# TheoBald200814/RGB-D-Instance-Segmentation

Hardware: AMD Instinct MI355X
Metric: NYUv2 640x480 RGB-D img/s (fwd+bwd) of the DGGM+E-DSAM hot path (higher is better)
Workload: dtype bf16

## Files before the change

rgb-d-instance-segmentation_amd/csrc/ratio_chain.hip:

```cpp
#include "ratio_common.hpp"

using namespace rgbd;
using namespace rgbd::rp;

namespace {

__global__ __launch_bounds__(256) void k_rp_fold(const char* __restrict__ blob, Layout L,
                                                 const float2* __restrict__ aff, int which, char* __restrict__ fold) {
  const int c = blockIdx.x;
  const int K = which == 1 ? STEM_K2 : STEM_C;
  const float* w = (const float*)(blob + (which == 1 ? L.w1f : L.w2f)) + (size_t)c * K;
  bf16_t* wo = (bf16_t*)(fold + (which == 1 ? FOLD_W1 : FOLD_W2)) + (size_t)c * K;
  const float2 a = aff[c];
  for (int k = threadIdx.x; k < K; k += 256) wo[k] = f32_to_bf16(w[k] * a.x);
  if (threadIdx.x == 0) {
    const float b = ((const float*)(blob + (which == 1 ? L.b1 : L.b2)))[c];
    ((float*)(fold + (which == 1 ? FOLD_B1 : FOLD_B2)))[c] = __builtin_fmaf(b, a.x, a.y);
  }
}

constexpr int C2W_PWP = 40;
constexpr size_t C2W_OFF_W1 = 0;
constexpr size_t C2W_OFF_W2 = C2W_OFF_W1 + (size_t)STEM_C * C2W_S1 * 2;
constexpr size_t C2W_OFF_W3 = C2W_OFF_W2 + (size_t)FUS_C * C2W_S2 * 2;
constexpr size_t C2W_OFF_W4 = C2W_OFF_W3 + (size_t)ATT_C * C2W_S3 * 2;
template <int PH> constexpr size_t c2w_off_b() {
  return PH == 0 ? C2W_OFF_W2 : C2W_OFF_W4 + (size_t)FUS_C * C2W_S4 * 2;
}
template <int PH> constexpr size_t c2w_off_aff() {
  return c2w_off_b<PH>() + (size_t)(STEM_C + FUS_C + ATT_C + FUS_C) * 4;
}
template <int PH> constexpr size_t c2w_off_patch() {
  return c2w_off_aff<PH>() + (size_t)(STEM_C + FUS_C) * 8;
}
template <int PH> constexpr size_t c2w_smem() { return c2w_off_patch<PH>() + (size_t)3 * C2W_PH * C2W_PWP * 2 + 16; }
static_assert(c2w_smem<1>() <= 163840, "chain v2 LDS budget");
constexpr size_t C2W_OFF_P8 = C2W_OFF_W3;
constexpr int C2W_P8 = 8 * 3 * C2W_PH * C2W_PWP;
static_assert(C2W_OFF_P8 + (size_t)C2W_P8 * 2 <= c2w_off_b<1>(), "phase-1 shifted patches fit W3 + W4");
static_assert(2 * c2w_smem<0>() <= 163840, "chain v2 phase 0: two workgroups per CU");

__device__ unsigned long long* g_c2_stamps = nullptr;
[[maybe_unused]] static bool c2_stamps_on = false;
__device__ __forceinline__ void c2_stamp(unsigned long long* st, long long idx) {
  __builtin_amdgcn_sched_barrier(0);
  const unsigned long long t = __builtin_amdgcn_s_memtime();
  if ((threadIdx.x & 63) == 0) st[idx] = t;
  __builtin_amdgcn_sched_barrier(0);
}

template <int PHASE, bool STAMPS = false>
__global__ __launch_bounds__(512, PHASE == 0 ? 4 : 2) void k_rp_chain_v2(const float* __restrict__ depth3, long long bstride, int B,
                                                     int H, int W, const char* __restrict__ blob, Layout L,
                                                     const float2* __restrict__ aff1, const float2* __restrict__ aff2,
                                                     const char* __restrict__ fold, float* __restrict__ slab,
                                                     bf16_t* __restrict__ att) {
  extern __shared__ __attribute__((aligned(16))) char smem[];
  const bf16_t* sW1 = (const bf16_t*)(smem + C2W_OFF_W1);
  const bf16_t* sW2 = (const bf16_t*)(smem + C2W_OFF_W2);
  const bf16_t* sW3 = (const bf16_t*)(smem + C2W_OFF_W3);
  const bf16_t* sW4 = (const bf16_t*)(smem + C2W_OFF_W4);
  float* sb = (float*)(smem + c2w_off_b<PHASE>());
  float* sb1 = sb;
  float* sb2 = sb1 + STEM_C;
  float* sb3 = sb2 + FUS_C;
  float* sb4 = sb3 + ATT_C;
  bf16_t* patch = (bf16_t*)(smem + c2w_off_patch<PHASE>());
  const int tid = threadIdx.x, lane = tid & 63, wave = tid >> 6;
  const int r = lane & 15, g = lane >> 4;
  {
    auto copy_rows = [&](size_t dst, size_t src, int rows, int k, int stride) {
      const int per = k / 8;
      for (int i = tid; i < rows * per; i += 512) {
        const int rr = i / per, q = i % per;
        *reinterpret_cast<uint4*>(smem + dst + ((size_t)rr * stride + 8 * q) * 2) =
            *reinterpret_cast<const uint4*>(blob + src + ((size_t)rr * k + 8 * q) * 2);
      }
    };
    auto copy_rows_p = [&](size_t dst, const char* base, int rows, int k, int stride) {
      const int per = k / 8;
      for (int i = tid; i < rows * per; i += 512) {
        const int rr = i / per, q = i % per;
        *reinterpret_cast<uint4*>(smem + dst + ((size_t)rr * stride + 8 * q) * 2) =
            *reinterpret_cast<const uint4*>(base + ((size_t)rr * k + 8 * q) * 2);
      }
    };
    if (PHASE == 0)
      copy_rows(C2W_OFF_W1, L.w1s, STEM_C, STEM_K2, C2W_S1);
    else
      copy_rows_p(C2W_OFF_W1, fold + FOLD_W1, STEM_C, STEM_K2, C2W_S1);
    if (PHASE >= 1) {
      if (PHASE == 2)
        copy_rows_p(C2W_OFF_W2, fold + FOLD_W2, FUS_C, STEM_C, C2W_S2);
      else
        copy_rows(C2W_OFF_W2, L.w2, FUS_C, STEM_C, C2W_S2);
    }
    if (PHASE == 2) {
      copy_rows(C2W_OFF_W3, L.w3, ATT_C, FUS_C, C2W_S3);
      copy_rows(C2W_OFF_W4, L.w4, FUS_C, ATT_C, C2W_S4);
    }
    for (int i = tid; i < STEM_C; i += 512)
      sb1[i] = PHASE == 0 ? ((const float*)(blob + L.b1))[i] : ((const float*)(fold + FOLD_B1))[i];
    for (int i = tid; i < FUS_C; i += 512)
      sb2[i] = PHASE == 2 ? ((const float*)(fold + FOLD_B2))[i] : ((const float*)(blob + L.b2))[i];
    for (int i = tid; i < ATT_C; i += 512) sb3[i] = ((const float*)(blob + L.b3))[i];
    for (int i = tid; i < FUS_C; i += 512) sb4[i] = ((const float*)(blob + L.b4))[i];
    for (int i = tid; i < 3 * C2W_PH * C2W_PWP; i += 512) patch[i] = 0;
    for (int i = tid; i < STEM_C * (C2W_S1 - STEM_K2); i += 512)
      ((bf16_t*)(smem + C2W_OFF_W1))[(i / (C2W_S1 - STEM_K2)) * C2W_S1 + STEM_K2 + i % (C2W_S1 - STEM_K2)] = 0;
  }
  constexpr int NST = PHASE == 0 ? 12 : 8;
  float ssum[NST], ssq[NST];
#pragma unroll
  for (int i = 0; i < NST; ++i) ssum[i] = ssq[i] = 0.f;
  const int tiles_x = (W + C2W_TW - 1) / C2W_TW, tiles_y = (H + C2W_TH - 1) / C2W_TH;
  const unsigned per = (unsigned)(tiles_x * tiles_y);
  const int ntiles = B * tiles_x * tiles_y;
  const long long HW = (long long)H * W;
  constexpr int PATCH_N = 3 * C2W_PH * C2W_PW, PATCH_PER = (PATCH_N + 511) / 512;
  float pre[PATCH_PER];
  const long long dbytes = ((long long)(B - 1) * bstride + 3 * HW) * 4;
  const bool dbuf = PHASE >= 1 && dbytes < (1ll << 31);
  const __amdgpu_buffer_rsrc_t drs = wt_rsrc(depth3, dbuf ? (int)dbytes : 0);
  auto fetch_patch = [&](int t) {
    const TileDec td = tile_dec((unsigned)t, per, (unsigned)tiles_x, C2W_TH, C2W_TW);
#pragma unroll
    for (int k = 0; k < PATCH_PER; ++k) {
      const int i = tid + 512 * k;
      const int c = i / (C2W_PH * C2W_PW), yy = (i / C2W_PW) % C2W_PH, xx = i % C2W_PW;
      const int yv = td.y0 + yy - 3, xv = td.x0 + xx - 3;
      const bool ok = i < PATCH_N && t < ntiles && yv >= 0 && yv < H && xv >= 0 && xv < W;
      if (dbuf) {
        const uint32_t off = ok ? (uint32_t)((td.b * bstride + c * HW + (long long)yv * W + xv) * 4) : 0x80000000u;
        pre[k] = __uint_as_float(__builtin_amdgcn_raw_buffer_load_b32(drs, off, 0, 0));
      } else {
        float v = 0.f;
        if (ok) v = depth3[td.b * bstride + c * HW + (long long)yv * W + xv];
        pre[k] = v;
      }
    }
  };
  auto add_stats = [&](float& sm, float& sq, const f32x4 (&a)[2], bool full, int x0, bool row_ok) {
#pragma unroll
    for (int u = 0; u < 2; ++u)
#pragma unroll
      for (int j = 0; j < 4; ++j) {
        float v = a[u][j];
        if (!full) v = (row_ok && x0 + 16 * u + 4 * g + j < W) ? v : 0.f;
        sm += v;
        sq = __builtin_fmaf(v, v, sq);
      }
  };
  fetch_patch(blockIdx.x);
  int tcount = 0;
  for (int tile = blockIdx.x; tile < ntiles; tile += gridDim.x, ++tcount) {
    unsigned long long* const sts = (STAMPS && blockIdx.x == 0 && tcount >= 8 && tcount < 12) ? g_c2_stamps : nullptr;
    const long long sidx = ((long long)PHASE * 32 + (long long)(tcount - 8) * 8 + wave) * 7;
    if (STAMPS && sts) c2_stamp(sts, sidx + 0);
    const TileDec td = tile_dec((unsigned)tile, per, (unsigned)tiles_x, C2W_TH, C2W_TW);
    const int b = td.b, y0 = td.y0, x0 = td.x0;
    lds_barrier();
#pragma unroll
    for (int k = 0; k < PATCH_PER; ++k) {
      const int i = tid + 512 * k;
      if (i < PATCH_N) patch[(i / C2W_PW) * C2W_PWP + i % C2W_PW] = f32_to_bf16(pre[k]);
    }
    lds_barrier();
    if constexpr (PHASE == 1) {
      bf16_t* p8 = (bf16_t*)(smem + C2W_OFF_P8);
      for (int i = tid; i < 8 * 3 * C2W_PH * 4; i += 512) {
        const int j8 = i & 3, row = (i >> 2) % (3 * C2W_PH), k = i / (3 * C2W_PH * 4);
        const int e = 8 * j8 + k;
        const uint32_t* wp = reinterpret_cast<const uint32_t*>(patch + row * C2W_PWP + (e & ~1));
        const uint32_t w0 = wp[0], w1 = wp[1], w2 = wp[2], w3 = wp[3], w4 = wp[4];
        const uint32_t sh = (e & 1) * 2;
        *reinterpret_cast<uint4*>(p8 + (k * 3 * C2W_PH + row) * C2W_PWP + 8 * j8) =
            make_uint4(__builtin_amdgcn_alignbyte(w1, w0, sh), __builtin_amdgcn_alignbyte(w2, w1, sh),
                       __builtin_amdgcn_alignbyte(w3, w2, sh), __builtin_amdgcn_alignbyte(w4, w3, sh));
      }
      lds_barrier();
    }
    if (STAMPS && sts) c2_stamp(sts, sidx + 1);
    fetch_patch(tile + gridDim.x);
    if (STAMPS && sts) c2_stamp(sts, sidx + 2);
    const int py = y0 + wave;
    const bool row_ok = py < H;
    const bool full = row_ok && x0 + C2W_TW <= W;
    bool pv[2];
#pragma unroll
    for (int u = 0; u < 2; ++u) pv[u] = row_ok && x0 + 16 * u + r < W;
    auto stem_b = [&](int s, Frag<bf16_t> (&bf)[2]) {
      const int q = 4 * s + g;
      if constexpr (PHASE == 1) {
        const int qc = q < 21 ? q : 20;
        const int cq = qc / 7, dy = qc - 7 * cq;
        const bf16_t* p8 = (const bf16_t*)(smem + C2W_OFF_P8) + (((r & 7) * 3 + cq) * C2W_PH + wave + dy) * C2W_PWP +
                           (r & 8);
        bf[0].v = *reinterpret_cast<const uint4*>(p8);
        bf[1].v = *reinterpret_cast<const uint4*>(p8 + 16);
        if (q >= 21) {
          bf[0].zero();
          bf[1].zero();
        }
        return;
      }
      const int cq = q / 7, dy = q - 7 * cq;
#pragma unroll
      for (int u = 0; u < 2; ++u) {
        if (q < 21) {
          const int col = 16 * u + r;
          const uint32_t* wp = reinterpret_cast<const uint32_t*>(patch + (cq * C2W_PH + wave + dy) * C2W_PWP + (col & ~1));
          const uint32_t w0 = wp[0], w1 = wp[1], w2 = wp[2], w3 = wp[3], w4 = wp[4];
          const uint32_t sh = (col & 1) * 2;
          bf[u].v = make_uint4(__builtin_amdgcn_alignbyte(w1, w0, sh), __builtin_amdgcn_alignbyte(w2, w1, sh),
                               __builtin_amdgcn_alignbyte(w3, w2, sh), __builtin_amdgcn_alignbyte(w4, w3, sh));
        } else {
          bf[u].zero();
        }
      }
    };
    auto stem_w = [&](int t, int s) {
      Frag<bf16_t> af;
      af.v = *reinterpret_cast<const uint4*>(sW1 + (16 * t + r) * C2W_S1 + 32 * s + 8 * g);
      if (s == 5) af.select(g == 0);
      return af;
    };
    auto stem_live = [](int t, int s) { return !((t < 4 && (s == 3 || s == 5)) || (t >= 4 && t < 8 && s == 5)); };
    if constexpr (PHASE == 0) {
      Frag<bf16_t> bfr[6][2];
#pragma unroll
      for (int s = 0; s < 6; ++s) stem_b(s, bfr[s]);
#pragma unroll
      for (int t = 0; t < 12; ++t) {
        const float bb = sb1[16 * t + r];
        f32x4 a1[2] = {f32x4{bb, bb, bb, bb}, f32x4{bb, bb, bb, bb}};
#pragma unroll
        for (int s = 0; s < 6; ++s) {
          if (!stem_live(t, s)) continue;
          const Frag<bf16_t> af = stem_w(t, s);
          mma(a1[0], bfr[s][0], af);
          mma(a1[1], bfr[s][1], af);
        }
        add_stats(ssum[t], ssq[t], a1, full, x0, row_ok);
      }
      if (STAMPS && sts) c2_stamp(sts, sidx + 3);
      continue;
    }
    f32x4 a1[12][2];
#pragma unroll
    for (int t = 0; t < 12; ++t) {
      const float4 bb = *reinterpret_cast<const float4*>(sb1 + 16 * t + 4 * g);
      a1[t][0] = a1[t][1] = f32x4{bb.x, bb.y, bb.z, bb.w};
    }
    if constexpr (PHASE == 1) {
      Frag<bf16_t> bcur[2], bnxt[2];
      stem_b(0, bcur);
#pragma unroll
      for (int s = 0; s < 6; ++s) {
        if (s < 5) stem_b(s + 1, bnxt);
#pragma unroll
        for (int t = 0; t < 12; ++t) {
          if (!stem_live(t, s)) continue;
          const Frag<bf16_t> af = stem_w(t, s);
          mma(a1[t][0], af, bcur[0]);
          mma(a1[t][1], af, bcur[1]);
        }
        __builtin_amdgcn_sched_barrier(0);
        bcur[0] = bnxt[0];
        bcur[1] = bnxt[1];
      }
    } else {
#pragma unroll
      for (int s = 0; s < 6; ++s) {
        Frag<bf16_t> bfr[2];
        stem_b(s, bfr);
#pragma unroll
        for (int t = 0; t < 12; ++t) {
          if (!stem_live(t, s)) continue;
          const Frag<bf16_t> af = stem_w(t, s);
          mma(a1[t][0], af, bfr[0]);
          mma(a1[t][1], af, bfr[1]);
        }
      }
    }
    if (STAMPS && sts) c2_stamp(sts, sidx + 3);
    Frag<bf16_t> f1[6][2];
#pragma unroll
    for (int s = 0; s < 6; ++s)
#pragma unroll
      for (int u = 0; u < 2; ++u) {
        float vv[8];
#pragma unroll
        for (int e = 0; e < 8; ++e) vv[e] = fmaxf(a1[2 * s + (e >> 2)][u][e & 3], 0.f);
        f1[s][u].from8(vv);
      }
    if (STAMPS && sts) c2_stamp(sts, sidx + 4);
    f32x4 a2[8][2];
#pragma unroll
    for (int t = 0; t < 8; ++t) {
      if constexpr (PHASE == 1) {
        const float bb = sb2[16 * t + r];
        a2[t][0] = a2[t][1] = f32x4{bb, bb, bb, bb};
      } else {
        const float4 bb = *reinterpret_cast<const float4*>(sb2 + 16 * t + 4 * g);
        a2[t][0] = a2[t][1] = f32x4{bb.x, bb.y, bb.z, bb.w};
      }
#pragma unroll
      for (int s = 0; s < 6; ++s) {
        Frag<bf16_t> af;
        af.v = *reinterpret_cast<const uint4*>(sW2 + (16 * t + r) * C2W_S2 + 32 * s + 8 * g);
        if constexpr (PHASE == 1) {
          mma(a2[t][0], f1[s][0], af);
          mma(a2[t][1], f1[s][1], af);
        } else {
          mma(a2[t][0], af, f1[s][0]);
          mma(a2[t][1], af, f1[s][1]);
        }
      }
    }
    if (STAMPS && sts) c2_stamp(sts, sidx + 5);
    if constexpr (PHASE == 1) {
#pragma unroll
      for (int t = 0; t < 8; ++t) add_stats(ssum[t], ssq[t], a2[t], full, x0, row_ok);
      if (att) {
        bf16_t* ft = att + (((long long)tile * 8 + wave) * 16) * 256;
#pragma unroll
        for (int t = 0; t < 8; ++t)
          *reinterpret_cast<uint4*>(ft + (t * 64 + lane) * 8) =
              make_uint4(pack_bf16x2(a2[t][0][0], a2[t][0][1]), pack_bf16x2(a2[t][0][2], a2[t][0][3]),
                         pack_bf16x2(a2[t][1][0], a2[t][1][1]), pack_bf16x2(a2[t][1][2], a2[t][1][3]));
      }
      if (STAMPS && sts) c2_stamp(sts, sidx + 6);
      continue;
    }
    if constexpr (PHASE == 2) {
#pragma unroll
      for (int t = 0; t < 8; ++t)
#pragma unroll
        for (int j = 0; j < 4; ++j) {
          a2[t][0][j] = fmaxf(a2[t][0][j], 0.f);
          a2[t][1][j] = fmaxf(a2[t][1][j], 0.f);
        }
      Frag<bf16_t> f2[4][2];
#pragma unroll
      for (int s = 0; s < 4; ++s)
#pragma unroll
        for (int u = 0; u < 2; ++u) {
          float vv[8];
#pragma unroll
          for (int e = 0; e < 8; ++e) vv[e] = a2[2 * s + (e >> 2)][u][e & 3];
          f2[s][u].from8(vv);
        }
      f32x4 a3[4][2];
#pragma unroll
      for (int t = 0; t < 4; ++t) {
        const float4 bb = *reinterpret_cast<const float4*>(sb3 + 16 * t + 4 * g);
        a3[t][0] = a3[t][1] = f32x4{bb.x, bb.y, bb.z, bb.w};
#pragma unroll
        for (int s = 0; s < 4; ++s) {
          Frag<bf16_t> af;
          af.v = *reinterpret_cast<const uint4*>(sW3 + (16 * t + r) * C2W_S3 + 32 * s + 8 * g);
          mma(a3[t][0], af, f2[s][0]);
          mma(a3[t][1], af, f2[s][1]);
        }
      }
      Frag<bf16_t> f3[2][2];
#pragma unroll
      for (int s = 0; s < 2; ++s)
#pragma unroll
        for (int u = 0; u < 2; ++u) {
          float vv[8];
#pragma unroll
          for (int e = 0; e < 8; ++e) vv[e] = fmaxf(a3[2 * s + (e >> 2)][u][e & 3], 0.f);
          f3[s][u].from8(vv);
        }
#pragma unroll
      for (int t = 0; t < 8; ++t) {
        const float4 bb = *reinterpret_cast<const float4*>(sb4 + 16 * t + 4 * g);
        f32x4 a4[2] = {f32x4{bb.x, bb.y, bb.z, bb.w}, f32x4{bb.x, bb.y, bb.z, bb.w}};
#pragma unroll
        for (int s = 0; s < 2; ++s) {
          Frag<bf16_t> af;
          af.v = *reinterpret_cast<const uint4*>(sW4 + (16 * t + r) * C2W_S4 + 32 * s + 8 * g);
          mma(a4[0], af, f3[s][0]);
          mma(a4[1], af, f3[s][1]);
        }
#pragma unroll
        for (int u = 0; u < 2; ++u) {
          if (!pv[u]) continue;
          float o[4];
#pragma unroll
          for (int j = 0; j < 4; ++j) o[j] = a2[t][u][j] * sigmoid_fast(a4[u][j]);
          *reinterpret_cast<uint2*>(att + c4_att_idx(b, t >> 1, py, x0 + 16 * u + r, H, W) + 16 * (t & 1) + 4 * g) =
              make_uint2(pack_bf16x2(o[0], o[1]), pack_bf16x2(o[2], o[3]));
        }
      }
    }
  }
  if constexpr (PHASE < 2) {
    const long long row = (long long)blockIdx.x * 8 + wave;
    constexpr int NC = PHASE == 0 ? STEM_C : FUS_C;
#pragma unroll
    for (int t = 0; t < NST; ++t) {
      float a = ssum[t], q = ssq[t];
      a += __shfl_xor(a, 16);
      q += __shfl_xor(q, 16);
      a += __shfl_xor(a, 32);
      q += __shfl_xor(q, 32);
      if (g == 0) {
        const long long e = PHASE == 1 ? (long long)(16 * t + r) * (gridDim.x * 8) + row : row * NC + 16 * t + r;
        slab[e * 2 + 0] = a;
        slab[e * 2 + 1] = q;
      }
    }
  }
}

template <int PH>
int chain_launch(const float* depth3, long long bstride, int B, int H, int W, const char* blob, const Layout& L,
                 const float2* aff1, const float2* aff2, const char* fold, float* slab, bf16_t* att, hipStream_t s) {
  static const hipError_t attr = hipFuncSetAttribute((const void*)k_rp_chain_v2<PH>,
                                                     hipFuncAttributeMaxDynamicSharedMemorySize, (int)c2w_smem<PH>());
  if (attr != hipSuccess) return (int)attr;
  const int grid = chain_grid_v2(B, H, W, PH);
#ifdef RGBD_DIAG
  if constexpr (PH < 2) {
    if (c2_stamps_on) {
      static const hipError_t sattr = hipFuncSetAttribute(
          (const void*)k_rp_chain_v2<PH, true>, hipFuncAttributeMaxDynamicSharedMemorySize, (int)c2w_smem<PH>());
      (void)sattr;
      k_rp_chain_v2<PH, true><<<grid, 512, c2w_smem<PH>(), s>>>(depth3, bstride, B, H, W, blob, L, aff1, aff2, fold,
                                                               slab, att);
      return RGBD_OK;
    }
  }
#endif
  k_rp_chain_v2<PH><<<grid, 512, c2w_smem<PH>(), s>>>(depth3, bstride, B, H, W, blob, L, aff1, aff2, fold, slab, att);
  return RGBD_OK;
}

}

namespace rgbd::rp {

int chain_grid_v2(int B, int H, int W, int phase) {
  const long long nt = (long long)B * ((W + C2W_TW - 1) / C2W_TW) * ((H + C2W_TH - 1) / C2W_TH);
  return (int)std::min<long long>(nt, phase == 0 ? 512 : 256);
}

int fold_bn(const char* blob, const Layout& L, const float2* aff, int which, char* fold, hipStream_t s) {
  k_rp_fold<<<which == 1 ? STEM_C : FUS_C, 256, 0, s>>>(blob, L, aff, which, fold);
  return RGBD_OK;
}

int chain_v2(int phase, const float* depth3, long long bstride, int B, int H, int W, const char* blob, const Layout& L,
             const float2* aff1, const float2* aff2, const char* fold, float* slab, bf16_t* att, hipStream_t s) {
  if (phase == 0) return chain_launch<0>(depth3, bstride, B, H, W, blob, L, aff1, aff2, fold, slab, att, s);
  if (phase == 1) return chain_launch<1>(depth3, bstride, B, H, W, blob, L, aff1, aff2, fold, slab, att, s);
  TimerScope ts("rp_chain", s);
  return chain_launch<2>(depth3, bstride, B, H, W, blob, L, aff1, aff2, fold, slab, att, s);
}

}

#ifdef RGBD_DIAG
extern "C" int rgbd_debug_chain_stamps(void* buf) {
  unsigned long long* p = (unsigned long long*)buf;
  const hipError_t e = hipMemcpyToSymbol(HIP_SYMBOL(g_c2_stamps), &p, sizeof(p));
  if (e != hipSuccess) return (int)e;
  c2_stamps_on = p != nullptr;
  return RGBD_OK;
}
#endif
```

rgb-d-instance-segmentation_amd/csrc/ratio_conv5.hip:

```cpp
#include "ratio_common.hpp"

using namespace rgbd;
using namespace rgbd::rp;

namespace {

constexpr int GT_S = FUS_C + 8;
constexpr size_t GT_OFF_W3 = 0;
constexpr size_t GT_OFF_W4 = GT_OFF_W3 + (size_t)ATT_C * C2W_S3 * 2;
constexpr size_t GT_OFF_B = GT_OFF_W4 + (size_t)FUS_C * C2W_S4 * 2;
constexpr size_t GT_OFF_IMG = GT_OFF_B + (size_t)(ATT_C + FUS_C + 2 * FUS_C) * 4;
constexpr size_t GT_SMEM = GT_OFF_IMG + (size_t)8 * C2W_TW * GT_S * 2;
static_assert(GT_SMEM <= 163840, "gate LDS budget");

__global__ __launch_bounds__(512) void k_rp_gate(const bf16_t* __restrict__ fus, int B, int H, int W,
                                                 const char* __restrict__ blob, Layout L,
                                                 const float2* __restrict__ aff2, bf16_t* __restrict__ att) {
  extern __shared__ __attribute__((aligned(16))) char smem[];
  const bf16_t* sW3 = (const bf16_t*)(smem + GT_OFF_W3);
  const bf16_t* sW4 = (const bf16_t*)(smem + GT_OFF_W4);
  float* sb3 = (float*)(smem + GT_OFF_B);
  float* sb4 = sb3 + ATT_C;
  float2* saff = (float2*)(sb4 + FUS_C);
  const int tid = threadIdx.x, lane = tid & 63, wave = tid >> 6;
// ... 480 lines not shown
            const float lo = __uint_as_float(w[2 * h + e] << 16), hi = __uint_as_float(w[2 * h + e] & 0xffff0000u);
            acc[nh][h] += fmaxf(lo * af[nh][h].x + af[nh][h].y, 0.f);
            acc[nh][h] += fmaxf(hi * af[nh][h].x + af[nh][h].y, 0.f);
          }
      }
    }
  }
#pragma unroll
  for (int nh = 0; nh < 2; ++nh)
#pragma unroll
    for (int h = 0; h < 2; ++h) {
      float v = acc[nh][h];
      v += __shfl_xor(v, 16);
      v += __shfl_xor(v, 32);
      if (lane < 16) red[nh * 128 + 32 * np + 16 * h + r] = v;
    }
  __syncthreads();
  part[(((long long)b * 16 + reg) * POOL_SPLIT + sp) * C5 + t] = red[t];
}

__global__ __launch_bounds__(256) void k_rp_bn_relu_pool_v4_frag(const bf16_t* __restrict__ y, int H, int W,
                                                                 const float2* __restrict__ aff,
                                                                 float* __restrict__ part) {
  __shared__ float red[2][C5];
  const int b = blockIdx.y, reg = blockIdx.x / POOL_SPLIT, sp = blockIdx.x % POOL_SPLIT;
  const int i = reg / 4, j = reg % 4;
  const int cp = threadIdx.x & 127, ql = threadIdx.x >> 7;
  const int nh = cp >> 6, np = (cp >> 4) & 3, r = cp & 15, n0 = nh * 128 + 32 * np + r, n1 = n0 + 16;
  const int ya = (i * H) / 4, yb = ((i + 1) * H + 3) / 4, xa = (j * W) / 4, xb = ((j + 1) * W + 3) / 4;
  const int rows = yb - ya;
  const int r0 = ya + (rows * sp) / POOL_SPLIT, r1 = ya + (rows * (sp + 1)) / POOL_SPLIT;
  const int qa = xa >> 2, nq = ((xb + 3) >> 2) - qa;
  const int tiles_x = (W + C4_TW - 1) / C4_TW, tiles_y = (H + C4_TH - 1) / C4_TH;
  const float2 a0 = aff[n0], a1 = aff[n1];
  float s0 = 0.f, s1 = 0.f;
  constexpr int PU = 8;
  int yy = r0, k = ql;
  while (k >= nq) {
    k -= nq;
    ++yy;
  }
  while (yy < r1) {
    uint4 v[PU];
    int xqs[PU];
    bool ok[PU];
#pragma unroll
    for (int u = 0; u < PU; ++u) {
      ok[u] = yy < r1;
      const int ry = ok[u] ? yy : r1 - 1, xq = (qa + (ok[u] ? k : 0)) * 4;
      xqs[u] = xq;
      const long long tile = ((long long)b * tiles_y + ry / C4_TH) * tiles_x + xq / C4_TW;
      const int ly = ry % C4_TH, lx = xq % C4_TW;
      const int wave = ly >> 1, mi = (ly & 1) * 2 + (lx >> 4), g = (lx & 15) >> 2;
      v[u] = *reinterpret_cast<const uint4*>(y + (((((2 * tile + nh) * 8 + wave) * 4 + mi) * 4 + np) * 64 + g * 16 + r) * 8);
      k += 2;
      while (k >= nq) {
        k -= nq;
        ++yy;
      }
    }
#pragma unroll
    for (int u = 0; u < PU; ++u) {
      const uint32_t w0[4] = {v[u].x, v[u].y, v[u].z, v[u].w};
#pragma unroll
      for (int e = 0; e < 4; ++e) {
        const int xx = xqs[u] + e;
        if (ok[u] && xx >= xa && xx < xb) {
          const float c0 = bf16_to_f32((bf16_t)(e & 1 ? w0[e >> 1] >> 16 : w0[e >> 1] & 0xffff));
          const float c1 = bf16_to_f32((bf16_t)(e & 1 ? w0[2 + (e >> 1)] >> 16 : w0[2 + (e >> 1)] & 0xffff));
          s0 += fmaxf(c0 * a0.x + a0.y, 0.f);
          s1 += fmaxf(c1 * a1.x + a1.y, 0.f);
        }
      }
    }
  }
  red[ql][n0] = s0;
  red[ql][n1] = s1;
  __syncthreads();
  const int c = threadIdx.x;
  part[(((long long)b * 16 + reg) * POOL_SPLIT + sp) * C5 + c] = red[0][c] + red[1][c];
}

__global__ __launch_bounds__(256) void k_rp_pool_finish_v4(const float* __restrict__ ip, int B, int H, int W,
                                                           float* __restrict__ pooled) {
  const int b = blockIdx.y, reg = blockIdx.x, i = reg / 4, j = reg % 4, c = threadIdx.x;
  const int nh = c >> 7, cc = c & 127;
  const int rh = H >> 2, rw = W >> 2;
  const int tiles_x = W / C4_TW, tiles_y = (H + C4_TH - 1) / C4_TH;
  const int ty0 = (i * rh) / C4_TH, ty1 = ((i + 1) * rh - 1) / C4_TH;
  const int tx0 = (j * rw) / C4_TW, tx1 = ((j + 1) * rw - 1) / C4_TW;
  float s = 0.f;
  for (int ty = ty0; ty <= ty1; ++ty)
    for (int tx = tx0; tx <= tx1; ++tx) {
      const int slot = (i - (ty * C4_TH) / rh) * 2 + (j - (tx * C4_TW) / rw);
      const long long tile = ((long long)b * tiles_y + ty) * tiles_x + tx;
      s += ip[((2 * tile + nh) * 4 + slot) * 128 + cc];
    }
  pooled[((long long)b * C5 + c) * 16 + reg] = s / (float)(rh * rw);
}

__global__ __launch_bounds__(256) void k_c4_pad_zero(bf16_t* __restrict__ att, int H, int W) {
  c4_pad_body(att, H, W, blockIdx.x, blockIdx.y, gridDim.x);
}

inline int gate_grid(int B, int H, int W) {
  return (int)std::min<long long>((long long)B * ((W + 31) / 32) * ((H + 7) / 8), device_cus());
}

template <int MODE>
int conv5_launch(const bf16_t* att, int B, int H, int W, const char* blob, const Layout& L, const float2* aff5,
                 bf16_t* y, float* out, hipStream_t s) {
  static const hipError_t sattr = hipFuncSetAttribute((const void*)k_rp_conv5_v4<MODE>,
                                                      hipFuncAttributeMaxDynamicSharedMemorySize, (int)C4_SMEM);
  if (sattr != hipSuccess) return (int)sattr;
  const int gcv = conv4_grid(B, H, W);
  k_rp_conv5_v4<MODE><<<gcv, 512, C4_SMEM, s>>>(att, B, H, W, blob, L, aff5, y, out, gcv % 16 == 0);
  return RGBD_OK;
}

}

namespace rgbd::rp {

int gate(const bf16_t* fus, int B, int H, int W, const char* blob, const Layout& L, const float2* aff2, bf16_t* att,
         hipStream_t s) {
  TimerScope ts("rp_chain", s);
  static const hipError_t gattr =
      hipFuncSetAttribute((const void*)k_rp_gate, hipFuncAttributeMaxDynamicSharedMemorySize, (int)GT_SMEM);
  if (gattr != hipSuccess) return (int)gattr;
  k_rp_gate<<<gate_grid(B, H, W), 512, GT_SMEM, s>>>(fus, B, H, W, blob, L, aff2, att);
  return RGBD_OK;
}

int c4_pad_zero(bf16_t* att, int B, int H, int W, hipStream_t s) {
  k_c4_pad_zero<<<dim3(8, B * 4), 256, 0, s>>>(att, H, W);
  return RGBD_OK;
}

long long conv4_tiles(int B, int H, int W) {
  return (long long)B * ((W + C4_TW - 1) / C4_TW) * ((H + C4_TH - 1) / C4_TH);
}
int conv4_grid(int B, int H, int W) { return 2 * (int)std::min<long long>(conv4_tiles(B, H, W), device_cus() / 2); }
bool conv4_pool_fused(int H, int W) { return H % 4 == 0 && W % 64 == 0 && H >= 64 && W >= 128; }

int conv5_v4(int mode, const bf16_t* att, int B, int H, int W, const char* blob, const Layout& L, const float2* aff5,
             bf16_t* y, float* out, hipStream_t s) {
  TimerScope ts("rp_conv3x3", s);
  return mode == 0   ? conv5_launch<0>(att, B, H, W, blob, L, aff5, y, out, s)
         : mode == 1 ? conv5_launch<1>(att, B, H, W, blob, L, aff5, y, out, s)
                     : conv5_launch<2>(att, B, H, W, blob, L, aff5, y, out, s);
}

int pool_v4(const bf16_t* y, int B, int H, int W, const float2* aff5, float* part, hipStream_t s) {
  if (H % 32 == 0 && W % 128 == 0)
    k_rp_bn_relu_pool_v4_tiles<<<dim3(16 * POOL_SPLIT, B), 256, 0, s>>>(y, H, W, aff5, part);
  else
    k_rp_bn_relu_pool_v4_frag<<<dim3(16 * POOL_SPLIT, B), 256, 0, s>>>(y, H, W, aff5, part);
  return RGBD_OK;
}

int pool_finish_v4(const float* ip, int B, int H, int W, float* pooled, hipStream_t s) {
  k_rp_pool_finish_v4<<<dim3(16, B), 256, 0, s>>>(ip, B, H, W, pooled);
  return RGBD_OK;
}

}

#ifdef RGBD_DIAG
extern "C" int rgbd_debug_conv5_stamps(void* buf) {
  unsigned long long* p = (unsigned long long*)buf;
  return (int)hipMemcpyToSymbol(HIP_SYMBOL(g_c4_stamps), &p, sizeof(p));
}
#endif
```

Baseline: 3205.

## Software-pipeline phase-1 chain kernel with double-buffered shifted patches and incremental tile decode

Gives phase 1 of the chain kernel its own loop. Depth patches are staged into double-buffered LDS (a plain copy and then a row-pair shifted layout) one or two tiles ahead, so the staging and the next global fetch overlap with the current tile's stem and fuse MMAs. Patch offsets are precomputed per thread and tile positions advance incrementally instead of being decoded by division each step, and stem MMAs now loop over s outermost with the B fragment prefetched. This trades extra LDS and register pressure, plus more complex indexing, for fewer barriers and less shift work per tile. Timer scopes are also added for phase 1 and pool.

```diff
diff --git a/rgb-d-instance-segmentation_amd/csrc/ratio_chain.hip b/rgb-d-instance-segmentation_amd/csrc/ratio_chain.hip
--- a/rgb-d-instance-segmentation_amd/csrc/ratio_chain.hip
+++ b/rgb-d-instance-segmentation_amd/csrc/ratio_chain.hip
@@ -35,9 +35,13 @@
 }
 template <int PH> constexpr size_t c2w_smem() { return c2w_off_patch<PH>() + (size_t)3 * C2W_PH * C2W_PWP * 2 + 16; }
 static_assert(c2w_smem<1>() <= 163840, "chain v2 LDS budget");
-constexpr size_t C2W_OFF_P8 = C2W_OFF_W3;
-constexpr int C2W_P8 = 8 * 3 * C2W_PH * C2W_PWP;
-static_assert(C2W_OFF_P8 + (size_t)C2W_P8 * 2 <= c2w_off_b<1>(), "phase-1 shifted patches fit W3 + W4");
+constexpr int C2W_S4_DW = (3 * C2W_PH / 2) * 9 * 16;
+constexpr int C2W_PP_EL = 3 * C2W_PH * C2W_PWP;
+constexpr size_t C2W_OFF_S4 = C2W_OFF_W3;
+constexpr size_t C2W_OFF_PP = C2W_OFF_S4 + 2 * (size_t)C2W_S4_DW * 4;
+static_assert((3 * C2W_PH) % 2 == 0 && 4 * 8 + 3 + 3 < C2W_PWP, "row pairs; chunk 8 of copy 3 ends inside the padded row");
+static_assert(C2W_OFF_S4 % 16 == 0 && C2W_OFF_PP % 16 == 0, "16-byte stores");
+static_assert(C2W_OFF_PP + 2 * (size_t)C2W_PP_EL * 2 <= c2w_off_b<1>(), "phase-1 patch buffers fit W3 + W4");
 static_assert(2 * c2w_smem<0>() <= 163840, "chain v2 phase 0: two workgroups per CU");
 
 __device__ unsigned long long* g_c2_stamps = nullptr;
@@ -106,6 +110,8 @@
     for (int i = tid; i < ATT_C; i += 512) sb3[i] = ((const float*)(blob + L.b3))[i];
     for (int i = tid; i < FUS_C; i += 512) sb4[i] = ((const float*)(blob + L.b4))[i];
     for (int i = tid; i < 3 * C2W_PH * C2W_PWP; i += 512) patch[i] = 0;
+    if constexpr (PHASE == 1)
+      for (int i = tid; i < 2 * C2W_PP_EL; i += 512) ((bf16_t*)(smem + C2W_OFF_PP))[i] = 0;
     for (int i = tid; i < STEM_C * (C2W_S1 - STEM_K2); i += 512)
       ((bf16_t*)(smem + C2W_OFF_W1))[(i / (C2W_S1 - STEM_K2)) * C2W_S1 + STEM_K2 + i % (C2W_S1 - STEM_K2)] = 0;
   }
@@ -151,125 +157,291 @@
         sq = __builtin_fmaf(v, v, sq);
       }
   };
-  fetch_patch(blockIdx.x);
-  int tcount = 0;
-  for (int tile = blockIdx.x; tile < ntiles; tile += gridDim.x, ++tcount) {
-    unsigned long long* const sts = (STAMPS && blockIdx.x == 0 && tcount >= 8 && tcount < 12) ? g_c2_stamps : nullptr;
-    const long long sidx = ((long long)PHASE * 32 + (long long)(tcount - 8) * 8 + wave) * 7;
-    if (STAMPS && sts) c2_stamp(sts, sidx + 0);
-    const TileDec td = tile_dec((unsigned)tile, per, (unsigned)tiles_x, C2W_TH, C2W_TW);
-    const int b = td.b, y0 = td.y0, x0 = td.x0;
+  auto stem_w = [&](int t, int s) {
+    Frag<bf16_t> af;
+    af.v = *reinterpret_cast<const uint4*>(sW1 + (16 * t + r) * C2W_S1 + 32 * s + 8 * g);
+    if (s == 5) af.select(g == 0);
+    return af;
+  };
+  auto stem_live = [](int t, int s) { return !((t < 4 && (s == 3 || s == 5)) || (t >= 4 && t < 8 && s == 5)); };
+  if constexpr (PHASE == 1) {
+    uint32_t* const s4 = (uint32_t*)(smem + C2W_OFF_S4);
+    bf16_t* const pp = (bf16_t*)(smem + C2W_OFF_PP);
+    constexpr int PLANE = C2W_PH * C2W_PW, REST = PLANE - 512;
+    static_assert(PATCH_PER == 4 && REST > 0 && 3 * REST <= 512 && 512 / C2W_PW == C2W_PH - 1, "phase-1 patch mapping");
+    const uint32_t chan4 = (uint32_t)(HW * 4);
+    uint32_t poff_a, pk_a, poff_b, pk_b;
+    {
+      const int yy = tid / C2W_PW, xx = tid % C2W_PW;
+      poff_a = (uint32_t)(((long long)(yy - 3) * W + (xx - 3)) * 4);
+      pk_a = (uint32_t)(yy * C2W_PWP + xx) | (uint32_t)yy << 11 | (uint32_t)xx << 15;
+      const int c = tid / REST, yb = C2W_PH - 1, xb = 512 + tid % REST - yb * C2W_PW;
+      const bool in = tid < 3 * REST;
+      poff_b = in ? (uint32_t)((c * HW + (long long)(yb - 3) * W + (xb - 3)) * 4) : 0x80000000u;
+      pk_b = in ? (uint32_t)((c * C2W_PH + yb) * C2W_PWP + xb) | (uint32_t)yb << 11 | (uint32_t)xb << 15 : 0u;
+    }
+    constexpr int S4_ITEMS = C2W_S4_DW / 4;
+    static_assert(S4_ITEMS <= 1024 && C2W_PWP == 40, "two pieces per thread; 20-dword patch rows");
+    uint32_t ssrc;
+    {
+      const int kp = tid & 1, par = (tid >> 1) & 1, m = (tid >> 2) % 9, rp = (tid >> 2) / 9;
+      ssrc = (uint32_t)((2 * rp + par) * 20 + 2 * m + kp) | (m >= 7 ? 1u << 15 : 0u);
+    }
+    const uint32_t lc = (uint32_t)((r >> 2) * 16 + (r & 3) * 2);
+    struct Pos {
+      int b, ty, tx;
+    };
+    const unsigned gs = gridDim.x;
+    const int step_b = (int)(gs / per), step_y = (int)((gs - step_b * per) / (unsigned)tiles_x),
+              step_x = (int)(gs - step_b * per - step_y * (unsigned)tiles_x);
+    auto advance = [&](Pos& p) {
+      p.tx += step_x;
+      if (p.tx >= tiles_x) {
+        p.tx -= tiles_x;
+        ++p.ty;
+      }
+      p.ty += step_y;
+      if (p.ty >= tiles_y) {
+        p.ty -= tiles_y;
+        ++p.b;
+      }
+      p.b += step_b;
+    };
+    const TileDec td0 = tile_dec(blockIdx.x, per, (unsigned)tiles_x, 1, 1);
+    Pos cur{td0.b, td0.y0, td0.x0}, nxt = cur;
+    long long ft = blockIdx.x;
+    auto fetch1 = [&] {
+      const bool live = ft < ntiles;
+      const int fy0 = nxt.ty * C2W_TH, fx0 = nxt.tx * C2W_TW;
+      if (dbuf) {
+        const uint32_t org = (uint32_t)((nxt.b * bstride + (long long)fy0 * W + fx0) * 4);
+        const bool inner = live && fy0 >= 3 && fy0 + C2W_TH + 3 <= H && fx0 >= 3 && fx0 + C2W_TW + 3 <= W;
+        uint32_t off[PATCH_PER];
+        off[0] = org + poff_a;
+        off[3] = org + poff_b;
+        if (!inner) {
+          const int ya = fy0 + (int)((pk_a >> 11) & 15) - 3, xa = fx0 + (int)(pk_a >> 15) - 3;
+          const int yb = fy0 + (int)((pk_b >> 11) & 15) - 3, xb = fx0 + (int)(pk_b >> 15) - 3;
+          if (!(live && (unsigned)ya < (unsigned)H && (unsigned)xa < (unsigned)W)) off[0] = 0x80000000u;
+          if (!(live && (unsigned)yb < (unsigned)H && (unsigned)xb < (unsigned)W)) off[3] = 0x80000000u;
+        }
+        off[1] = off[0] + chan4;
+        off[2] = off[1] + chan4;
+#pragma unroll
+        for (int k = 0; k < PATCH_PER; ++k)
+          pre[k] = __uint_as_float(__builtin_amdgcn_raw_buffer_load_b32(drs, off[k], 0, 0));
+      } else if (live) {
+        long long hw = HW;
+        asm volatile("" : "+s"(hw));
+        const float* img = depth3 + nxt.b * bstride;
+#pragma unroll
+        for (int k = 0; k < PATCH_PER; ++k) {
+          const uint32_t pk = k < 3 ? pk_a : pk_b;
+          const int c = k < 3 ? k : tid / REST;
+          const int yv = fy0 + (int)((pk >> 11) & 15) - 3, xv = fx0 + (int)(pk >> 15) - 3;
+          float v = 0.f;
+          if ((k < 3 || tid < 3 * REST) && yv >= 0 && yv < H && xv >= 0 && xv < W) v = img[c * hw + (long long)yv * W + xv];
+          pre[k] = v;
+        }
+      }
+      advance(nxt);
+      ft += gs;
+    };
+    auto stage_plain = [&](int buf) {
+      bf16_t* p = pp + buf * C2W_PP_EL;
+#pragma unroll
+      for (int k = 0; k < 3; ++k) p[(pk_a & 0x7ffu) + k * C2W_PH * C2W_PWP] = f32_to_bf16(pre[k]);
+      if (tid < 3 * REST) p[pk_b & 0x7ffu] = f32_to_bf16(pre[3]);
+    };
+    auto stage_shift = [&](int buf) {
+      const uint32_t* p = reinterpret_cast<const uint32_t*>(pp + buf * C2W_PP_EL);
+      uint32_t* d = s4 + buf * C2W_S4_DW;
+#pragma unroll
+      for (int j = 0; j < 2; ++j) {
+        const int i = tid + 512 * j;
+        const uint32_t sj = (ssrc & 0x7fffu) + (j ? 564u + 22u * (ssrc >> 15) : 0u);
+        if (i < S4_ITEMS) {
+          const uint32_t w0 = p[sj], w1 = p[sj + 1], w2 = p[sj + 2];
+          *reinterpret_cast<uint4*>(d + 4 * i) =
+              make_uint4(w0, w1, __builtin_amdgcn_alignbyte(w1, w0, 2), __builtin_amdgcn_alignbyte(w2, w1, 2));
+        }
+      }
+    };
+    fetch1();
     lds_barrier();
-#pragma unroll
-    for (int k = 0; k < PATCH_PER; ++k) {
-      const int i = tid + 512 * k;
-      if (i < PATCH_N) patch[(i / C2W_PW) * C2W_PWP + i % C2W_PW] = f32_to_bf16(pre[k]);
-    }
+    stage_plain(0);
+    fetch1();
     lds_barrier();
-    if constexpr (PHASE == 1) {
-      bf16_t* p8 = (bf16_t*)(smem + C2W_OFF_P8);
-      for (int i = tid; i < 8 * 3 * C2W_PH * 4; i += 512) {
-        const int j8 = i & 3, row = (i >> 2) % (3 * C2W_PH), k = i / (3 * C2W_PH * 4);
-        const int e = 8 * j8 + k;
-        const uint32_t* wp = reinterpret_cast<const uint32_t*>(patch + row * C2W_PWP + (e & ~1));
-        const uint32_t w0 = wp[0], w1 = wp[1], w2 = wp[2], w3 = wp[3], w4 = wp[4];
-        const uint32_t sh = (e & 1) * 2;
-        *reinterpret_cast<uint4*>(p8 + (k * 3 * C2W_PH + row) * C2W_PWP + 8 * j8) =
-            make_uint4(__builtin_amdgcn_alignbyte(w1, w0, sh), __builtin_amdgcn_alignbyte(w2, w1, sh),
-                       __builtin_amdgcn_alignbyte(w3, w2, sh), __builtin_amdgcn_alignbyte(w4, w3, sh));
-      }
+    stage_shift(0);
+    stage_plain(1);
+    fetch1();
+    int tcount = 0;
+    for (int tile = blockIdx.x; tile < ntiles; tile += gridDim.x, ++tcount) {
+      unsigned long long* const sts = (STAMPS && blockIdx.x == 0 && tcount >= 8 && tcount < 12) ? g_c2_stamps : nullptr;
+      const long long sidx = ((long long)PHASE * 32 + (long long)(tcount - 8) * 8 + wave) * 7;
+      if (STAMPS && sts) c2_stamp(sts, sidx + 0);
+      const int cb = tcount & 1;
+      const int y0 = cur.ty * C2W_TH, x0 = cur.tx * C2W_TW;
+      advance(cur);
       lds_barrier();
-    }
-    if (STAMPS && sts) c2_stamp(sts, sidx + 1);
-    fetch_patch(tile + gridDim.x);
-    if (STAMPS && sts) c2_stamp(sts, sidx + 2);
-    const int py = y0 + wave;
-    const bool row_ok = py < H;
-    const bool full = row_ok && x0 + C2W_TW <= W;
-    bool pv[2];
-#pragma unroll
-    for (int u = 0; u < 2; ++u) pv[u] = row_ok && x0 + 16 * u + r < W;
-    auto stem_b = [&](int s, Frag<bf16_t> (&bf)[2]) {
-      const int q = 4 * s + g;
-      if constexpr (PHASE == 1) {
+      if (STAMPS && sts) c2_stamp(sts, sidx + 1);
+      const int py = y0 + wave;
+      const bool row_ok = py < H;
+      const bool full = row_ok && x0 + C2W_TW <= W;
+      const uint32_t* sbuf = s4 + cb * C2W_S4_DW;
+      auto stem_b = [&](int s, Frag<bf16_t> (&bf)[2]) {
+        const int q = 4 * s + g;
         const int qc = q < 21 ? q : 20;
-        const int cq = qc / 7, dy = qc - 7 * cq;
-        const bf16_t* p8 = (const bf16_t*)(smem + C2W_OFF_P8) + (((r & 7) * 3 + cq) * C2W_PH + wave + dy) * C2W_PWP +
-                           (r & 8);
-        bf[0].v = *reinterpret_cast<const uint4*>(p8);
-        bf[1].v = *reinterpret_cast<const uint4*>(p8 + 16);
+        const int row = qc + 7 * ((qc >= 7) + (qc >= 14)) + wave;
+        uint32_t a[4];
+#pragma unroll
+        for (int e = 0; e < 4; ++e) {
+          a[e] = (uint32_t)((row >> 1) * 144 + (row & 1) * 8) + lc + (uint32_t)((e >> 1) * 64 + (e & 1) * 16);
+          asm("" : "+v"(a[e]));
+        }
+        const uint2 v0 = *reinterpret_cast<const uint2*>(sbuf + a[0]), v1 = *reinterpret_cast<const uint2*>(sbuf + a[1]);
+        const uint2 v2 = *reinterpret_cast<const uint2*>(sbuf + a[2]), v3 = *reinterpret_cast<const uint2*>(sbuf + a[3]);
+        bf[0].v = make_uint4(v0.x, v0.y, v1.x, v1.y);
+        bf[1].v = make_uint4(v2.x, v2.y, v3.x, v3.y);
         if (q >= 21) {
           bf[0].zero();
           bf[1].zero();
         }
-        return;
-      }
-      const int cq = q / 7, dy = q - 7 * cq;
-#pragma unroll
-      for (int u = 0; u < 2; ++u) {
-        if (q < 21) {
-          const int col = 16 * u + r;
-          const uint32_t* wp = reinterpret_cast<const uint32_t*>(patch + (cq * C2W_PH + wave + dy) * C2W_PWP + (col & ~1));
-          const uint32_t w0 = wp[0], w1 = wp[1], w2 = wp[2], w3 = wp[3], w4 = wp[4];
-          const uint32_t sh = (col & 1) * 2;
-          bf[u].v = make_uint4(__builtin_amdgcn_alignbyte(w1, w0, sh), __builtin_amdgcn_alignbyte(w2, w1, sh),
-                               __builtin_amdgcn_alignbyte(w3, w2, sh), __builtin_amdgcn_alignbyte(w4, w3, sh));
-        } else {
-          bf[u].zero();
-        }
-      }
-    };
-    auto stem_w = [&](int t, int s) {
-      Frag<bf16_t> af;
-      af.v = *reinterpret_cast<const uint4*>(sW1 + (16 * t + r) * C2W_S1 + 32 * s + 8 * g);
-      if (s == 5) af.select(g == 0);
-      return af;
-    };
-    auto stem_live = [](int t, int s) { return !((t < 4 && (s == 3 || s == 5)) || (t >= 4 && t < 8 && s == 5)); };
-    if constexpr (PHASE == 0) {
-      Frag<bf16_t> bfr[6][2];
-#pragma unroll
-      for (int s = 0; s < 6; ++s) stem_b(s, bfr[s]);
+      };
+      f32x4 a1[12][2];
 #pragma unroll
       for (int t = 0; t < 12; ++t) {
-        const float bb = sb1[16 * t + r];
-        f32x4 a1[2] = {f32x4{bb, bb, bb, bb}, f32x4{bb, bb, bb, bb}};
+        const float4 bb = *reinterpret_cast<const float4*>(sb1 + 16 * t + 4 * g);
+        a1[t][0] = a1[t][1] = f32x4{bb.x, bb.y, bb.z, bb.w};
+      }
+      {
+        Frag<bf16_t> bcur[2], bnxt[2];
+        stem_b(0, bcur);
 #pragma unroll
         for (int s = 0; s < 6; ++s) {
-          if (!stem_live(t, s)) continue;
-          const Frag<bf16_t> af = stem_w(t, s);
-          mma(a1[0], bfr[s][0], af);
-          mma(a1[1], bfr[s][1], af);
-        }
-        add_stats(ssum[t], ssq[t], a1, full, x0, row_ok);
-      }
+          if (s < 5) stem_b(s + 1, bnxt);
+#pragma unroll
+          for (int t = 0; t < 12; ++t) {
+            if (!stem_live(t, s)) continue;
+            const Frag<bf16_t> af = stem_w(t, s);
+            mma(a1[t][0], af, bcur[0]);
+            mma(a1[t][1], af, bcur[1]);
+          }
+          __builtin_amdgcn_sched_barrier(0);
+          bcur[0] = bnxt[0];
+          bcur[1] = bnxt[1];
+        }
+      }
+      if (STAMPS && sts) c2_stamp(sts, sidx + 2);
+      Frag<bf16_t> f1[6][2];
+#pragma unroll
+      for (int s = 0; s < 6; ++s)
+#pragma unroll
+        for (int u = 0; u < 2; ++u) {
+          float vv[8];
+#pragma unroll
+          for (int e = 0; e < 8; ++e) vv[e] = fmaxf(a1[2 * s + (e >> 2)][u][e & 3], 0.f);
+          f1[s][u].from8(vv);
+        }
       if (STAMPS && sts) c2_stamp(sts, sidx + 3);
-      continue;
-    }
-    f32x4 a1[12][2];
-#pragma unroll
-    for (int t = 0; t < 12; ++t) {
-      const float4 bb = *reinterpret_cast<const float4*>(sb1 + 16 * t + 4 * g);
-      a1[t][0] = a1[t][1] = f32x4{bb.x, bb.y, bb.z, bb.w};
-    }
-    if constexpr (PHASE == 1) {
-      Frag<bf16_t> bcur[2], bnxt[2];
-      stem_b(0, bcur);
-#pragma unroll
-      for (int s = 0; s < 6; ++s) {
-        if (s < 5) stem_b(s + 1, bnxt);
+      if ((long long)tile + 2 * (long long)gs < ntiles) stage_plain(cb);
+      fetch1();
+      if ((long long)tile + gs < ntiles) stage_shift(cb ^ 1);
+      if (STAMPS && sts) c2_stamp(sts, sidx + 4);
+      f32x4 a2[8][2];
+#pragma unroll
+      for (int t = 0; t < 8; ++t) {
+        const float bb = sb2[16 * t + r];
+        a2[t][0] = a2[t][1] = f32x4{bb, bb, bb, bb};
+#pragma unroll
+        for (int s = 0; s < 6; ++s) {
+          Frag<bf16_t> af;
+          af.v = *reinterpret_cast<const uint4*>(sW2 + (16 * t + r) * C2W_S2 + 32 * s + 8 * g);
+          mma(a2[t][0], f1[s][0], af);
+          mma(a2[t][1], f1[s][1], af);
+        }
+      }
+      if (STAMPS && sts) c2_stamp(sts, sidx + 5);
+#pragma unroll
+      for (int t = 0; t < 8; ++t) add_stats(ssum[t], ssq[t], a2[t], full, x0, row_ok);
+      if (att) {
+        bf16_t* ft_out = att + (((long long)tile * 8 + wave) * 16) * 256;
+#pragma unroll
+        for (int t = 0; t < 8; ++t)
+          *reinterpret_cast<uint4*>(ft_out + (t * 64 + lane) * 8) =
+              make_uint4(pack_bf16x2(a2[t][0][0], a2[t][0][1]), pack_bf16x2(a2[t][0][2], a2[t][0][3]),
+                         pack_bf16x2(a2[t][1][0], a2[t][1][1]), pack_bf16x2(a2[t][1][2], a2[t][1][3]));
+      }
+      if (STAMPS && sts) c2_stamp(sts, sidx + 6);
+    }
+  } else {
+    fetch_patch(blockIdx.x);
+    int tcount = 0;
+    for (int tile = blockIdx.x; tile < ntiles; tile += gridDim.x, ++tcount) {
+      unsigned long long* const sts = (STAMPS && blockIdx.x == 0 && tcount >= 8 && tcount < 12) ? g_c2_stamps : nullptr;
+      const long long sidx = ((long long)PHASE * 32 + (long long)(tcount - 8) * 8 + wave) * 7;
+      if (STAMPS && sts) c2_stamp(sts, sidx + 0);
+      const TileDec td = tile_dec((unsigned)tile, per, (unsigned)tiles_x, C2W_TH, C2W_TW);
+      const int b = td.b, y0 = td.y0, x0 = td.x0;
+      lds_barrier();
+#pragma unroll
+      for (int k = 0; k < PATCH_PER; ++k) {
+        const int i = tid + 512 * k;
+        if (i < PATCH_N) patch[(i / C2W_PW) * C2W_PWP + i % C2W_PW] = f32_to_bf16(pre[k]);
+      }
+      lds_barrier();
+      if (STAMPS && sts) c2_stamp(sts, sidx + 1);
+      fetch_patch(tile + gridDim.x);
+      if (STAMPS && sts) c2_stamp(sts, sidx + 2);
+      const int py = y0 + wave;
+      const bool row_ok = py < H;
+      const bool full = row_ok && x0 + C2W_TW <= W;
+      bool pv[2];
+#pragma unroll
+      for (int u = 0; u < 2; ++u) pv[u] = row_ok && x0 + 16 * u + r < W;
+      auto stem_b = [&](int s, Frag<bf16_t> (&bf)[2]) {
+        const int q = 4 * s + g;
+        const int cq = q / 7, dy = q - 7 * cq;
+#pragma unroll
+        for (int u = 0; u < 2; ++u) {
+          if (q < 21) {
+            const int col = 16 * u + r;
+            const uint32_t* wp = reinterpret_cast<const uint32_t*>(patch + (cq * C2W_PH + wave + dy) * C2W_PWP + (col & ~1));
+            const uint32_t w0 = wp[0], w1 = wp[1], w2 = wp[2], w3 = wp[3], w4 = wp[4];
+            const uint32_t sh = (col & 1) * 2;
+            bf[u].v = make_uint4(__builtin_amdgcn_alignbyte(w1, w0, sh), __builtin_amdgcn_alignbyte(w2, w1, sh),
+                                 __builtin_amdgcn_alignbyte(w3, w2, sh), __builtin_amdgcn_alignbyte(w4, w3, sh));
+          } else {
+            bf[u].zero();
+          }
+        }
+      };
+      if constexpr (PHASE == 0) {
+        Frag<bf16_t> bfr[6][2];
+#pragma unroll
+        for (int s = 0; s < 6; ++s) stem_b(s, bfr[s]);
 #pragma unroll
         for (int t = 0; t < 12; ++t) {
-          if (!stem_live(t, s)) continue;
-          const Frag<bf16_t> af = stem_w(t, s);
-          mma(a1[t][0], af, bcur[0]);
-          mma(a1[t][1], af, bcur[1]);
-        }
-        __builtin_amdgcn_sched_barrier(0);
-        bcur[0] = bnxt[0];
-        bcur[1] = bnxt[1];
-      }
-    } else {
+          const float bb = sb1[16 * t + r];
+          f32x4 a1[2] = {f32x4{bb, bb, bb, bb}, f32x4{bb, bb, bb, bb}};
+#pragma unroll
+          for (int s = 0; s < 6; ++s) {
+            if (!stem_live(t, s)) continue;
+            const Frag<bf16_t> af = stem_w(t, s);
+            mma(a1[0], bfr[s][0], af);
+            mma(a1[1], bfr[s][1], af);
+          }
+          add_stats(ssum[t], ssq[t], a1, full, x0, row_ok);
+        }
+        if (STAMPS && sts) c2_stamp(sts, sidx + 3);
+        continue;
+      }
+      f32x4 a1[12][2];
+#pragma unroll
+      for (int t = 0; t < 12; ++t) {
+        const float4 bb = *reinterpret_cast<const float4*>(sb1 + 16 * t + 4 * g);
+        a1[t][0] = a1[t][1] = f32x4{bb.x, bb.y, bb.z, bb.w};
+      }
 #pragma unroll
       for (int s = 0; s < 6; ++s) {
         Frag<bf16_t> bfr[2];
@@ -282,117 +454,90 @@
           mma(a1[t][1], af, bfr[1]);
         }
       }
-    }
-    if (STAMPS && sts) c2_stamp(sts, sidx + 3);
-    Frag<bf16_t> f1[6][2];
-#pragma unroll
-    for (int s = 0; s < 6; ++s)
-#pragma unroll
-      for (int u = 0; u < 2; ++u) {
-        float vv[8];
-#pragma unroll
-        for (int e = 0; e < 8; ++e) vv[e] = fmaxf(a1[2 * s + (e >> 2)][u][e & 3], 0.f);
-        f1[s][u].from8(vv);
-      }
-    if (STAMPS && sts) c2_stamp(sts, sidx + 4);
-    f32x4 a2[8][2];
-#pragma unroll
-    for (int t = 0; t < 8; ++t) {
-      if constexpr (PHASE == 1) {
-        const float bb = sb2[16 * t + r];
-        a2[t][0] = a2[t][1] = f32x4{bb, bb, bb, bb};
-      } else {
+      Frag<bf16_t> f1[6][2];
+#pragma unroll
+      for (int s = 0; s < 6; ++s)
+#pragma unroll
+        for (int u = 0; u < 2; ++u) {
+          float vv[8];
+#pragma unroll
+          for (int e = 0; e < 8; ++e) vv[e] = fmaxf(a1[2 * s + (e >> 2)][u][e & 3], 0.f);
+          f1[s][u].from8(vv);
+        }
+      f32x4 a2[8][2];
+#pragma unroll
+      for (int t = 0; t < 8; ++t) {
         const float4 bb = *reinterpret_cast<const float4*>(sb2 + 16 * t + 4 * g);
         a2[t][0] = a2[t][1] = f32x4{bb.x, bb.y, bb.z, bb.w};
-      }
-#pragma unroll
-      for (int s = 0; s < 6; ++s) {
-        Frag<bf16_t> af;
-        af.v = *reinterpret_cast<const uint4*>(sW2 + (16 * t + r) * C2W_S2 + 32 * s + 8 * g);
-        if constexpr (PHASE == 1) {
-          mma(a2[t][0], f1[s][0], af);
-          mma(a2[t][1], f1[s][1], af);
-        } else {
+#pragma unroll
+        for (int s = 0; s < 6; ++s) {
+          Frag<bf16_t> af;
+          af.v = *reinterpret_cast<const uint4*>(sW2 + (16 * t + r) * C2W_S2 + 32 * s + 8 * g);
           mma(a2[t][0], af, f1[s][0]);
           mma(a2[t][1], af, f1[s][1]);
         }
       }
-    }
-    if (STAMPS && sts) c2_stamp(sts, sidx + 5);
-    if constexpr (PHASE == 1) {
-#pragma unroll
-      for (int t = 0; t < 8; ++t) add_stats(ssum[t], ssq[t], a2[t], full, x0, row_ok);
-      if (att) {
-        bf16_t* ft = att + (((long long)tile * 8 + wave) * 16) * 256;
+      if constexpr (PHASE == 2) {
 #pragma unroll
         for (int t = 0; t < 8; ++t)
-          *reinterpret_cast<uint4*>(ft + (t * 64 + lane) * 8) =
-              make_uint4(pack_bf16x2(a2[t][0][0], a2[t][0][1]), pack_bf16x2(a2[t][0][2], a2[t][0][3]),
-                         pack_bf16x2(a2[t][1][0], a2[t][1][1]), pack_bf16x2(a2[t][1][2], a2[t][1][3]));
-      }
-      if (STAMPS && sts) c2_stamp(sts, sidx + 6);
-      continue;
-    }
-    if constexpr (PHASE == 2) {
-#pragma unroll
-      for (int t = 0; t < 8; ++t)
-#pragma unroll
-        for (int j = 0; j < 4; ++j) {
-          a2[t][0][j] = fmaxf(a2[t][0][j], 0.f);
-          a2[t][1][j] = fmaxf(a2[t][1][j], 0.f);
-        }
-      Frag<bf16_t> f2[4][2];
-#pragma unroll
-      for (int s = 0; s < 4; ++s)
-#pragma unroll
-        for (int u = 0; u < 2; ++u) {
-          float vv[8];
-#pragma unroll
-          for (int e = 0; e < 8; ++e) vv[e] = a2[2 * s + (e >> 2)][u][e & 3];
-          f2[s][u].from8(vv);
-        }
-      f32x4 a3[4][2];
-#pragma unroll
-      for (int t = 0; t < 4; ++t) {
-        const float4 bb = *reinterpret_cast<const float4*>(sb3 + 16 * t + 4 * g);
-        a3[t][0] = a3[t][1] = f32x4{bb.x, bb.y, bb.z, bb.w};
-#pragma unroll
-        for (int s = 0; s < 4; ++s) {
-          Frag<bf16_t> af;
-          af.v = *reinterpret_cast<const uint4*>(sW3 + (16 * t + r) * C2W_S3 + 32 * s + 8 * g);
-          mma(a3[t][0], af, f2[s][0]);
-          mma(a3[t][1], af, f2[s][1]);
-        }
-      }
-      Frag<bf16_t> f3[2][2];
-#pragma unroll
-      for (int s = 0; s < 2; ++s)
-#pragma unroll
-        for (int u = 0; u < 2; ++u) {
-          float vv[8];
-#pragma unroll
-          for (int e = 0; e < 8; ++e) vv[e] = fmaxf(a3[2 * s + (e >> 2)][u][e & 3], 0.f);
-          f3[s][u].from8(vv);
-        }
-#pragma unroll
-      for (int t = 0; t < 8; ++t) {
-        const float4 bb = *reinterpret_cast<const float4*>(sb4 + 16 * t + 4 * g);
-        f32x4 a4[2] = {f32x4{bb.x, bb.y, bb.z, bb.w}, f32x4{bb.x, bb.y, bb.z, bb.w}};
-#pragma unroll
-        for (int s = 0; s < 2; ++s) {
-          Frag<bf16_t> af;
-          af.v = *reinterpret_cast<const uint4*>(sW4 + (16 * t + r) * C2W_S4 + 32 * s + 8 * g);
-          mma(a4[0], af, f3[s][0]);
-          mma(a4[1], af, f3[s][1]);
-        }
-#pragma unroll
-        for (int u = 0; u < 2; ++u) {
-          if (!pv[u]) continue;
-          float o[4];
-#pragma unroll
-          for (int j = 0; j < 4; ++j) o[j] = a2[t][u][j] * sigmoid_fast(a4[u][j]);
-          *reinterpret_cast<uint2*>(att + c4_att_idx(b, t >> 1, py, x0 + 16 * u + r, H, W) + 16 * (t & 1) + 4 * g) =
-              make_uint2(pack_bf16x2(o[0], o[1]), pack_bf16x2(o[2], o[3]));
+#pragma unroll
+          for (int j = 0; j < 4; ++j) {
+            a2[t][0][j] = fmaxf(a2[t][0][j], 0.f);
+            a2[t][1][j] = fmaxf(a2[t][1][j], 0.f);
+          }
+        Frag<bf16_t> f2[4][2];
+#pragma unroll
+        for (int s = 0; s < 4; ++s)
+#pragma unroll
+          for (int u = 0; u < 2; ++u) {
+            float vv[8];
+#pragma unroll
+            for (int e = 0; e < 8; ++e) vv[e] = a2[2 * s + (e >> 2)][u][e & 3];
+            f2[s][u].from8(vv);
+          }
+        f32x4 a3[4][2];
+#pragma unroll
+        for (int t = 0; t < 4; ++t) {
+          const float4 bb = *reinterpret_cast<const float4*>(sb3 + 16 * t + 4 * g);
+          a3[t][0] = a3[t][1] = f32x4{bb.x, bb.y, bb.z, bb.w};
+#pragma unroll
+          for (int s = 0; s < 4; ++s) {
+            Frag<bf16_t> af;
+            af.v = *reinterpret_cast<const uint4*>(sW3 + (16 * t + r) * C2W_S3 + 32 * s + 8 * g);
+            mma(a3[t][0], af, f2[s][0]);
+            mma(a3[t][1], af, f2[s][1]);
+          }
+        }
+        Frag<bf16_t> f3[2][2];
+#pragma unroll
+        for (int s = 0; s < 2; ++s)
+#pragma unroll
+          for (int u = 0; u < 2; ++u) {
+            float vv[8];
+#pragma unroll
+            for (int e = 0; e < 8; ++e) vv[e] = fmaxf(a3[2 * s + (e >> 2)][u][e & 3], 0.f);
+            f3[s][u].from8(vv);
+          }
+#pragma unroll
+        for (int t = 0; t < 8; ++t) {
+          const float4 bb = *reinterpret_cast<const float4*>(sb4 + 16 * t + 4 * g);
+          f32x4 a4[2] = {f32x4{bb.x, bb.y, bb.z, bb.w}, f32x4{bb.x, bb.y, bb.z, bb.w}};
+#pragma unroll
+          for (int s = 0; s < 2; ++s) {
+            Frag<bf16_t> af;
+            af.v = *reinterpret_cast<const uint4*>(sW4 + (16 * t + r) * C2W_S4 + 32 * s + 8 * g);
+            mma(a4[0], af, f3[s][0]);
+            mma(a4[1], af, f3[s][1]);
+          }
+#pragma unroll
+          for (int u = 0; u < 2; ++u) {
+            if (!pv[u]) continue;
+            float o[4];
+#pragma unroll
+            for (int j = 0; j < 4; ++j) o[j] = a2[t][u][j] * sigmoid_fast(a4[u][j]);
+            *reinterpret_cast<uint2*>(att + c4_att_idx(b, t >> 1, py, x0 + 16 * u + r, H, W) + 16 * (t & 1) + 4 * g) =
+                make_uint2(pack_bf16x2(o[0], o[1]), pack_bf16x2(o[2], o[3]));
+          }
         }
       }
     }
@@ -456,7 +601,10 @@
 int chain_v2(int phase, const float* depth3, long long bstride, int B, int H, int W, const char* blob, const Layout& L,
              const float2* aff1, const float2* aff2, const char* fold, float* slab, bf16_t* att, hipStream_t s) {
   if (phase == 0) return chain_launch<0>(depth3, bstride, B, H, W, blob, L, aff1, aff2, fold, slab, att, s);
-  if (phase == 1) return chain_launch<1>(depth3, bstride, B, H, W, blob, L, aff1, aff2, fold, slab, att, s);
+  if (phase == 1) {
+    TimerScope ts("rp_chain_p1", s);
+    return chain_launch<1>(depth3, bstride, B, H, W, blob, L, aff1, aff2, fold, slab, att, s);
+  }
   TimerScope ts("rp_chain", s);
   return chain_launch<2>(depth3, bstride, B, H, W, blob, L, aff1, aff2, fold, slab, att, s);
 }
diff --git a/rgb-d-instance-segmentation_amd/csrc/ratio_conv5.hip b/rgb-d-instance-segmentation_amd/csrc/ratio_conv5.hip
--- a/rgb-d-instance-segmentation_amd/csrc/ratio_conv5.hip
+++ b/rgb-d-instance-segmentation_amd/csrc/ratio_conv5.hip
@@ -656,6 +656,7 @@
 }
 
 int pool_v4(const bf16_t* y, int B, int H, int W, const float2* aff5, float* part, hipStream_t s) {
+  TimerScope ts("rp_pool", s);
   if (H % 32 == 0 && W % 128 == 0)
     k_rp_bn_relu_pool_v4_tiles<<<dim3(16 * POOL_SPLIT, B), 256, 0, s>>>(y, H, W, aff5, part);
   else
```

After: 3234 (median of 6 runs). Within noise of the previous version (+0.9%).
